# zlib-ng/minizip-ng

Measured on NVIDIA H100. Metric: deflate_l1_crc32_input_throughput, higher is better.
Workload: dtype u8

## Files before the change

minizip-ng_b200/csrc/deflate_kernel.cuh:

```cuda
#ifndef MZ_DEFLATE_KERNEL_CUH
#define MZ_DEFLATE_KERNEL_CUH

#include "mzcuda_common.cuh"

namespace mzc {

constexpr int DF_THREADS = 512;
constexpr int DF_WARPS = DF_THREADS / 32;
constexpr int DF_CHUNK_MAX = 65536;
constexpr int DF_UNIT = 32768;
constexpr int DF_SB = DF_UNIT;
constexpr int DF_SPAN = 8;
constexpr int DF_BATCH = DF_THREADS * DF_SPAN;
constexpr int DF_NBATCH = DF_UNIT / DF_BATCH;
constexpr int DF_MINMATCH = 4;
constexpr int DF_LOCKLEN = 8;
constexpr int DF_HASH_BITS = 13;
constexpr int DF_HASH_ENTRIES = 1 << DF_HASH_BITS;
constexpr int DF_STAGE_WORDS = DF_UNIT / 4 + 64;
constexpr int DF_HDR_WORDS = 96;

constexpr uint32_t DF_FLAG_FINAL = 1u;
constexpr uint32_t DF_FLAG_DICT = 2u;

constexpr int DF_OFF_IN = 0;
constexpr int DF_OFF_HASH = DF_OFF_IN + DF_UNIT + 64;
constexpr int DF_OFF_STAGE = DF_OFF_HASH;
constexpr int DF_OFF_REC = DF_OFF_HASH + DF_STAGE_WORDS * 4;
constexpr int DF_OFF_SPN = DF_OFF_REC + DF_NBATCH * DF_THREADS * 8;
constexpr int DF_SPAN_BYTES = DF_NBATCH * DF_THREADS * 10;
constexpr int DF_OFF_HIST = DF_OFF_REC + DF_SPAN_BYTES;
constexpr int DF_OFF_HIST2 = DF_OFF_HIST + (288 + 32) * 4;
constexpr int DF_OFF_CODE = DF_OFF_HIST2 + 256 * 4;
constexpr int DF_OFF_LENS = DF_OFF_CODE + (288 + 32) * 4;
constexpr int DF_OFF_BITS = DF_OFF_LENS + (288 + 32);
constexpr int DF_OFF_SCAN = DF_OFF_BITS + (288 + 32);
constexpr int DF_OFF_BB = DF_OFF_SCAN + 256 * 4;
constexpr int DF_OFF_MISC = DF_OFF_BB + 512 * 4;
constexpr int DF_OFF_SINK = DF_OFF_MISC + 32 * 4 + 16;
constexpr int DF_OFF_LSYM = DF_OFF_SINK + 32 * 4;
constexpr int DF_SMEM_BYTES = DF_OFF_LSYM + 256 * 2;
constexpr int DF_OFF_CAPL = DF_OFF_HIST;
static_assert(DF_OFF_CAPL + DF_WARPS * DF_NBATCH * 32 <= DF_OFF_SCAN, "capped-span lists fit in front of the scan scratch");
constexpr uint32_t DF_ZERO_SYM = 286;
static_assert(DF_HASH_ENTRIES * 4 <= DF_STAGE_WORDS * 4, "hash fits the staging region");
constexpr int DFH_PREV = 32768;
constexpr int DFH_HASH_BITS = 14;
constexpr int DFH_OFF_HASH = (DF_SMEM_BYTES + 15) & ~15;
constexpr int DFH_SMEM_BYTES = DFH_PREV + DFH_OFF_HASH + (4 << DFH_HASH_BITS);
static_assert(DFH_SMEM_BYTES <= 227 * 1024, "shared memory budget of the history variant");
static_assert(DF_SMEM_BYTES <= 113 * 1024, "shared memory budget for two CTAs per SM");

enum { MISC_CHUNK = 3, MISC_CARRY = 8  };

struct DeflateParams {
    const uint8_t *in;
    const uint64_t *in_off;
    const uint32_t *in_len;
    const uint8_t *flags;
    uint64_t total_len;
    uint32_t chunk_size;
    uint32_t nchunks;
    uint32_t last_flags;
    int32_t level;
    uint8_t *out;
    uint64_t slot_stride;
    uint32_t *out_len;
    uint32_t *work_counter;
};

__host__ __device__ inline uint64_t deflate_slot_bound(uint32_t chunk_size) {
    return (((uint64_t)chunk_size + 12ull * ((chunk_size + DF_SB - 1) / DF_SB + 1) + 64 + 15) & ~15ull);
}

__device__ __forceinline__ void length_symbol(uint32_t len, uint32_t &sym, uint32_t &ebits, uint32_t &eval) {
    const uint32_t l = len - 3;
    const uint32_t msb = 31u - (uint32_t)__clz((int)(l | 4u));
    uint32_t e = msb - 2;
    uint32_t sy = 4 * (e + 1) + ((l >> e) & 3u);
    uint32_t ev = l & ((1u << e) - 1u);
    sy = l < 8 ? l : sy;
    const bool top = len == 258;
    sym = top ? 28u : sy;
    ebits = top ? 0u : e;
    eval = top ? 0u : ev;
}
__device__ __forceinline__ void dist_symbol0(uint32_t d, uint32_t &sym, uint32_t &ebits) {
    uint32_t m = 31u - (uint32_t)__clz((int)(d | 1u));
    ebits = m > 0 ? m - 1 : 0u;
    sym = 2 * m + ((d >> ebits) & 1u);
}
__device__ __forceinline__ uint32_t len_extra_bits(uint32_t lsym) { return (lsym < 8 || lsym >= 28) ? 0u : (lsym >> 2) - 1; }
__device__ __forceinline__ uint32_t dist_extra_bits(uint32_t dsym) { return dsym < 4 ? 0u : (dsym >> 1) - 1; }

__device__ __forceinline__ uint32_t stage_word(uint32_t base, uint32_t pos, uint32_t k4) { return base + __umulhi(pos, 1u << 27) * k4; }

__device__ __forceinline__ void stage_put(uint32_t *stage, uint32_t pos, uint32_t v, uint32_t n) {
    if (n == 0) return;
    if (n < 32) v &= (1u << n) - 1;
    uint32_t w = pos >> 5, s = pos & 31;
    atomicOr(&stage[w], v << s);
    if (s + n > 32) atomicOr(&stage[w + 1], v >> (32 - s));
}

__device__ __forceinline__ void stage_or(const Smem &sm, uint32_t pos, uint32_t v, uint32_t n) {
    const uint32_t sh = pos & 31u, wa = DF_OFF_STAGE + ((pos >> 5) << 2);
    sm.red_or32(wa, v << sh);
    if (sh + n > 32) sm.red_or32(wa + 4, v >> (32 - sh));
}

struct BitWriter {
    Smem sm;
    uint64_t acc;
    uint32_t nb, wa;
    __device__ __forceinline__ void init(const Smem &s, uint32_t bitoff) {
        sm = s; wa = DF_OFF_STAGE + (bitoff >> 5) * 4; nb = bitoff & 31; acc = 0;
    }
    __device__ __forceinline__ void put(uint32_t v, uint32_t n) {
        acc |= (uint64_t)v << nb;
        nb += n;
        if (nb >= 32) {
            sm.red_or32(wa, (uint32_t)acc);
            acc >>= 32; nb -= 32; wa += 4;
        }
    }
    __device__ __forceinline__ uint32_t bitpos() const { return ((wa - (uint32_t)DF_OFF_STAGE) << 3) + nb; }
    __device__ __forceinline__ void finish() {
        if (nb > 0) sm.red_or32(wa, (uint32_t)acc);
        if (nb > 32) sm.red_or32(wa + 4, (uint32_t)(acc >> 32));
    }
};

enum { DF_PH_LOAD, DF_PH_PARSE, DF_PH_M0, DF_PH_COVER, DF_PH_T_M1, DF_PH_D, DF_PH_EMIT, DF_PH_FLUSH, DF_PH_UNITS,
       DF_PH_D_STATS, DF_PH_D_SWEEP1, DF_PH_D_SWEEP2, DF_PH_D_KRAFT, DF_PH_D_CANON, DF_PH_D_PASSES,
       DF_PH_P_A = DF_PH_D_PASSES + 8, DF_PH_P_B, DF_PH_P_C, DF_PH_M_INDEX, DF_PH_M_NEAR, DF_PH_M_EXTEND, DF_PH_X_SCAN, DF_PH_X_EMIT,
       DF_PH_X_M3, DF_PH_COLS };
constexpr int DF_PH_ROWS = 1024;
#if defined(MZ_DF_PHASES) && !defined(MZ_EMU)
__device__ unsigned long long g_df_phases[DF_PH_ROWS][DF_PH_COLS];
#define DF_PHASE_BEGIN(t) unsigned long long t = clock64()
#define DF_PHASE(t, ph)                                                                        \
    do {                                                                                       \
        if (threadIdx.x == 0 && blockIdx.x < (unsigned)DF_PH_ROWS) {                           \
            const unsigned long long now_ = clock64();                                         \
            atomicAdd(&g_df_phases[blockIdx.x][ph], now_ - (t));                               \
            if ((ph) == DF_PH_LOAD) atomicAdd(&g_df_phases[blockIdx.x][DF_PH_UNITS], 1ull);   \
            (t) = now_;                                                                        \
        }                                                                                      \
    } while (0)
#define DF_PHASE_COUNT(col)                                                                                          \
    do {                                                                                                             \
        if (threadIdx.x == 0 && blockIdx.x < (unsigned)DF_PH_ROWS) atomicAdd(&g_df_phases[blockIdx.x][col], 1ull); \
    } while (0)
#else
#define DF_PHASE_BEGIN(t)
#define DF_PHASE(t, ph)
#define DF_PHASE_COUNT(col)
#endif

constexpr int DF_BB_THREADS = 320;
enum { BB_STAT = 0 , BB_KRAFT = 8 , BB_SLACK = 136 ,
       BB_CNTW = 144 ,
       BB_NZ = 464 , BB_ST = 474 ,
       BB_HSUM = 484 , BB_HDRBITS = 494 ,
       BB_TOKBITS = 495 , BB_TOKW = 496  };

constexpr uint64_t CL_LENS = 0x12ddad91b725bb4ull;
constexpr uint64_t CL_CODE_LO = 0x840013930ef3c6ull, CL_CODE_HI = 0xd5c7fdf6cb149ull;
constexpr uint64_t CL_ORDER57 = 0x1b6d6db248db92dull;
__device__ __forceinline__ uint32_t cl_len(uint32_t s) { return (uint32_t)(CL_LENS >> (3 * s)) & 7u; }
__device__ __forceinline__ uint32_t cl_code(uint32_t s) {
    return s < 10 ? (uint32_t)(CL_CODE_LO >> (6 * s)) & 63u : (uint32_t)(CL_CODE_HI >> (6 * (s - 10))) & 63u;
}

__device__ __forceinline__ void bb_count_lengths(uint32_t *cntw_row, uint32_t L, unsigned lane, unsigned &m) {
    if (lane < 16) cntw_row[lane] = 0;
    __syncwarp();
    m = __match_any_sync(MZ_FULL_MASK, L);
    if (L > 0 && lane == (unsigned)(__ffs((int)m) - 1)) cntw_row[L] = (uint32_t)__popc(m);
    __syncwarp();
}

__device__ inline void block_build_codes(const uint32_t *hist_ll, const uint32_t *hist_lit2, const uint32_t *hist_d, uint8_t *lens_ll, uint8_t *lens_d,
                                         uint32_t *code_ll, uint32_t *code_d, uint8_t *bits_ll, uint8_t *bits_d, uint32_t *bb,
                                         uint32_t *stage, uint32_t hdrpos, uint32_t bfinal) {
    const uint32_t tid = threadIdx.x;
    const unsigned lane = lane_id(), w = warp_id();
    const int a = tid < 288 ? 0 : (tid < 320 ? 1 : 2);
    const uint32_t sym = a == 0 ? tid : tid - 288;
    const uint32_t nsym = a == 0 ? 286u : 30u;
    const int M = 15;
    const uint32_t one = 1u << M;
    const uint32_t w0 = a == 0 ? 0u : 9u;
    uint32_t c = (a < 2 && sym < nsym) ? (a == 0 ? hist_ll[sym] + (sym < 256 ? hist_lit2[sym] : 0u) : hist_d[sym]) : 0u;
    DF_PHASE_BEGIN(d_t);

    if (tid < 144) bb[tid] = (tid == BB_STAT + 2 || tid == BB_STAT + 6) ? 0xffffffffu : 0u;
    bar_sync(1, DF_BB_THREADS);
    if (a < 2) {
        uint32_t used_w = __reduce_add_sync(MZ_FULL_MASK, c ? 1u : 0u);
        uint32_t tot_w = __reduce_add_sync(MZ_FULL_MASK, c);
        uint32_t first_w = __reduce_min_sync(MZ_FULL_MASK, c ? sym : 0xffffffffu);
        if (lane == 0) {
            atomicAdd(&bb[BB_STAT + a * 4 + 0], used_w);
            atomicAdd(&bb[BB_STAT + a * 4 + 1], tot_w);
            atomicMin(&bb[BB_STAT + a * 4 + 2], first_w);
        }
    }
    bar_sync(1, DF_BB_THREADS);
    DF_PHASE(d_t, DF_PH_D_STATS);
    float ideal = 0.f;
    if (a < 2) {
        uint32_t used = bb[BB_STAT + a * 4 + 0], total = bb[BB_STAT + a * 4 + 1], fu = bb[BB_STAT + a * 4 + 2];
        if (used < 2) {
            uint32_t d0 = used == 0 ? 0u : (fu == 0 ? 1u : 0u);
            uint32_t d1 = used == 0 ? 1u : d0;
            if ((sym == d0 || sym == d1) && c == 0) c = 1;
            total += 2 - used;
        }
        if (c) ideal = __log2f((float)total) - __log2f((float)c);
    }
    float lo = -3.0f, step = 0.25f;
    uint32_t slack[2] = {0, 0};
    for (int sweep = 0; sweep < 2; sweep++) {
        if (a < 2) {
            uint32_t mine = 0;
#pragma unroll
            for (int cnd = 0; cnd < 16; cnd++) {
                uint32_t kr = 0;
                if (c) {
                    int l = (int)ceilf(ideal - (lo + step * (float)cnd));
                    l = l < 1 ? 1 : (l > M ? M : l);
                    kr = 1u << (M - l);
                }
                kr = __reduce_add_sync(MZ_FULL_MASK, kr);
                mine = lane == (unsigned)cnd ? kr : mine;
            }
            if (lane < 16) atomicAdd(&bb[BB_KRAFT + sweep * 32 + a * 16 + lane], mine);
        }
        bar_sync(1, DF_BB_THREADS);
        DF_PHASE(d_t, DF_PH_D_SWEEP1 + sweep);
        const uint32_t kl = bb[BB_KRAFT + sweep * 32 + lane];
        const unsigned fit = __ballot_sync(MZ_FULL_MASK, (lane & 15u) != 0 && kl <= one);
        const int best0 = (fit & 0xffffu) ? 31 - __clz((int)(fit & 0xffffu)) : 0;
        const int best1 = (fit >> 16) ? 31 - __clz((int)(fit >> 16)) : 0;
        slack[0] = one - __shfl_sync(MZ_FULL_MASK, kl, best0);
        slack[1] = one - __shfl_sync(MZ_FULL_MASK, kl, 16 + best1);
        lo = lo + step * (float)(a == 0 ? best0 : best1);
        step *= 0.0625f;
    }
    uint32_t L = 0;
    if (c) {
        int l = (int)ceilf(ideal - lo);
        L = (uint32_t)(l < 1 ? 1 : (l > M ? M : l));
    }
    unsigned m = 0;
    int buf = 0, pass = 0;
    bool settled = false;
    for (; pass < 40; pass++) {
        if (slack[0] == 0 && slack[1] == 0) break;
        uint32_t *cntw = bb + BB_CNTW + buf * 160, *nxt = bb + BB_CNTW + (buf ^ 1) * 160;
        if (a < 2) bb_count_lengths(cntw + w * 16, L, lane, m);
        bar_sync(1, DF_BB_THREADS);
        if (w == 0 || w == 9) {
            const int aa = w == 0 ? 0 : 1;
            const uint32_t wa = aa == 0 ? 0u : 9u, wb = aa == 0 ? 9u : 10u;
            const bool mine = lane >= 1 && lane <= (unsigned)M;
            uint32_t P[9], tot = 0;
#pragma unroll
            for (int i = 0; i < 9; i++) {
                const uint32_t t = (mine && wa + i < wb) ? cntw[(wa + i) * 16 + lane] : 0u;
                P[i] = tot;
                tot += t;
            }
            uint32_t sl = slack[aa], myk = 0;
            for (int len = 2; len <= M; len++) {
                uint32_t t = __shfl_sync(MZ_FULL_MASK, tot, len);
                uint32_t can = sl >> (M - len);
                uint32_t k = t < can ? t : can;
                if (lane == (unsigned)len) myk = k;
                sl -= k << (M - len);
            }
            const uint32_t kup = __shfl_down_sync(MZ_FULL_MASK, myk, 1);
            const uint32_t tot2 = mine ? tot - myk + kup : 0u;
            uint32_t code = 0, prev = 0, mycode = 0;
            for (int len = 1; len <= M; len++) {
                code = (code + prev) << 1;
                if (lane == (unsigned)len) mycode = code;
                prev = __shfl_sync(MZ_FULL_MASK, tot2, len);
// ... 162 lines not shown
__device__ __forceinline__ uint32_t opaque4() { return blockDim.x / (uint32_t)(DF_THREADS / 4); }

template <bool HIST>
__device__ __forceinline__ uint32_t hash_addr(uint32_t v, uint32_t k4) {
    return (HIST ? DFH_OFF_HASH : DF_OFF_HASH) + __umulhi(v * 2654435761u, 1u << (HIST ? DFH_HASH_BITS : DF_HASH_BITS)) * k4;
}

__device__ __forceinline__ uint32_t rec_len(uint32_t r) { uint32_t l = (r >> 3) & 255u; return l ? l + 3 : 0u; }

__device__ __forceinline__ uint32_t fin_len(uint32_t m) { return ((m >> 4) & 255u) + 3u; }
__device__ __forceinline__ uint32_t fin_dist(uint32_t m) { return ((m >> 12) & 0x7fffu) + 1u; }
template <bool ONEM>
__device__ __forceinline__ void span_classify(const Smem &sm, uint32_t A, uint32_t B, uint32_t q0, uint32_t cover, uint32_t &F, uint32_t &MA,
                                              uint32_t &MB) {
    const uint32_t lit = (A >> 26) | ((B >> 26) << 6);
    const uint32_t crel = cover > q0 ? cover - q0 : 0u;
    const uint32_t cr8 = crel < 8 ? crel : 8u;
    uint32_t ex = 0;
    MA = MB = 0;
#pragma unroll
    for (int r = 0; r < (ONEM ? 1 : 2); r++) {
        const uint32_t R = r == 0 ? A : B;
        const uint32_t j = R & 7u, end = j + rec_len(R);
        const uint32_t s = j > crel ? j : crel;
        const uint32_t Lf = (end > s ? end : s) - s;
        const uint32_t P = (s < 8u ? s : 8u) & 7u;
        const uint32_t M = Lf >= 3 ? (((Lf << 4) + (0x80000000u - (3u << 4))) | P | ((R << 1) & (0x7fffu << 12))) : 0u;
        if (r == 0) MA = M;
        else MB = M;
        ex = Lf - 1u < 2u ? Lf : ex;
    }
    F = ((lit >> cr8) << cr8) | (ex << 8);
    if (ex) {
        const uint32_t p = DF_OFF_IN + q0 + crel;
        F |= sm.ld8(p) << 16;
        if (ex == 2) F |= sm.ld8(p + 1) << 24;
    }
}

__device__ __forceinline__ uint32_t match_symbols(const Smem &sm, uint32_t M) {
    uint32_t ds, db;
    const uint32_t lsv = sm.ld16(DF_OFF_LSYM + ((M >> 3) & 0x1feu));
    const uint32_t d = fin_dist(M) - 1;
    dist_symbol0(d, ds, db);
    sm.red_add32(DF_OFF_HIST + (257u + (lsv & 31u)) * 4, 1u);
    sm.red_add32(DF_OFF_HIST + (288u + ds) * 4, 1u);
    return 0x80000000u | ((M & 7u) << 28) | ((d & ((1u << db) - 1u)) << 15) | (ds << 10) | lsv;
}
__device__ __forceinline__ uint32_t match_bits(const Smem &sm, uint32_t M) {
    const uint32_t n = sm.ld8(DF_OFF_BITS + 257u + (M & 31u)) + sm.ld8(DF_OFF_BITS + 288u + ((M >> 10) & 31u));
    return M ? n : 0u;
}
__device__ __forceinline__ void put_match_bits(const Smem &sm, uint32_t pos, uint32_t M) {
    const uint32_t cwl = sm.ld32(DF_OFF_CODE + (257u + (M & 31u)) * 4);
    const uint32_t cwd = sm.ld32(DF_OFF_CODE + (288u + ((M >> 10) & 31u)) * 4);
    const uint32_t cl = (cwl >> 16) & 15u, cd = (cwd >> 16) & 15u;
    const uint32_t v1 = (cwl & 0x7fffu) | (((M >> 5) & 31u) << cl);
    const uint32_t n1 = cl + ((cwl >> 20) & 15u);
    const uint32_t v2 = (cwd & 0x7fffu) | (((M >> 15) & 0x1fffu) << cd);
    const uint64_t V = (uint64_t)v1 | ((uint64_t)v2 << n1);
    const uint32_t lo = (uint32_t)V, hi = (uint32_t)(V >> 32);
    const uint32_t wa = stage_word(DF_OFF_STAGE, pos, opaque4());
    const uint32_t w0 = __funnelshift_l(0u, lo, pos), w1 = __funnelshift_l(lo, hi, pos), w2 = __funnelshift_l(hi, 0u, pos);
    sm.red_or32(wa, w0);
    sm.red_or32(wa + 4, w1);
    if (w2) sm.red_or32(wa + 8, w2);
}

__device__ __forceinline__ uint32_t nth_parked(const uint32_t (&bm)[DF_NBATCH], uint32_t k, uint32_t warp) {
    uint32_t r = k, word = 0, bsel = 0;
    bool found = false;
#pragma unroll
    for (int b = 0; b < DF_NBATCH; b++) {
        const uint32_t c = (uint32_t)__popc(bm[b]);
        const bool here = !found && r < c;
        word = here ? bm[b] : word;
        bsel = here ? (uint32_t)b : bsel;
        found = found || here;
        r -= found ? 0u : c;
    }
    uint32_t base = 0;
#pragma unroll
    for (int st = 16; st; st >>= 1) {
        const uint32_t c = (uint32_t)__popc((word >> base) & ((1u << st) - 1u));
        const bool up = r >= c;
        r -= up ? c : 0u;
        base += up ? (uint32_t)st : 0u;
    }
    return found ? bsel * (uint32_t)DF_THREADS + warp * 32u + base : 0xffffffffu;
}

struct SpanBits {
    uint32_t v[4], E0, E1, offs, xv, MA, size;
};
template <bool ONEM>
__device__ __forceinline__ SpanBits span_bits(const Smem &sm, uint32_t sidx, uint32_t F, uint32_t MA, uint32_t MB, uint32_t code_base, uint32_t zero_ent,
                                              uint32_t k4) {
    SpanBits s;
    const uint2 x = sm.ld64(DF_OFF_IN + sidx * DF_SPAN);
    uint32_t xn = 0;
    s.xv = 0;
    const uint32_t ex = (F >> 8) & 3u;
    if (ex) {
        const uint32_t c0 = sm.ld32(DF_OFF_CODE + ((F >> 16) & 0xffu) * 4);
        s.xv = c0 & 0x7fffu;
        xn = (c0 >> 16) & 15u;
        if (ex == 2) {
            const uint32_t c1 = sm.ld32(DF_OFF_CODE + (F >> 24) * 4);
            s.xv |= (c1 & 0x7fffu) << xn;
            xn += (c1 >> 16) & 15u;
        }
    }
    uint32_t cw[8];
#pragma unroll
    for (int j = 0; j < 8; j++) {
        const uint32_t by = MZ_BYTE(j < 4 ? x.x : x.y, j & 3);
        cw[j] = sm.ld32_a(((F >> j) & 1u) ? by * k4 + code_base : zero_ent);
    }
    const uint32_t nA = match_bits(sm, MA), nB = ONEM ? 0u : match_bits(sm, MB);
    const uint32_t sA = MA ? ((MA >> 28) & 7u) * 8u : 64u, sB = MB ? ((MB >> 28) & 7u) * 8u : 64u;
    const uint32_t L0 = __byte_perm(__byte_perm(cw[0], cw[1], 0x0062u), __byte_perm(cw[2], cw[3], 0x0062u), 0x5410u) + shl_clamp(nA, sA) + shl_clamp(nB, sB);
    const uint32_t L1 = __byte_perm(__byte_perm(cw[4], cw[5], 0x0062u), __byte_perm(cw[6], cw[7], 0x0062u), 0x5410u) + shl_clamp(nA, sA - 32u) + shl_clamp(nB, sB - 32u);
    const uint32_t P0 = L0 * 0x01010101u;
    const uint32_t P1 = L1 * 0x01010101u + (P0 >> 24) * 0x01010101u;
    s.E0 = P0 << 8;
    s.E1 = __funnelshift_l(P0, P1, 8);
#pragma unroll
    for (int jj = 0; jj < 4; jj++) {
        const uint32_t c0 = cw[2 * jj], c1 = cw[2 * jj + 1];
        s.v[jj] = (c0 & 0xffffu) | ((c1 & 0xffffu) << (c0 >> 16));
    }
    s.offs = xn + (((shr_clamp(s.E0, sA) & 0xffu) + (shr_clamp(s.E1, sA - 32u) & 0xffu)) << 8) +
             (((shr_clamp(s.E0, sB) & 0xffu) + (shr_clamp(s.E1, sB - 32u) & 0xffu)) << 16);
    s.MA = MA;
    s.size = xn + (P1 >> 24);
    return s;
}
template <bool ONEM>
__device__ __forceinline__ void span_emit(const Smem &sm, const SpanBits &s, uint32_t pos, uint32_t sidx, uint32_t stage_base, uint32_t k4) {
    const uint32_t xn = s.offs & 0xffu;
    if (xn) stage_or(sm, pos, s.xv, xn);
    pos += xn;
#pragma unroll
    for (int jj = 0; jj < 4; jj++) {
        const uint32_t pp = pos + MZ_BYTE(jj < 2 ? s.E0 : s.E1, 2 * (jj & 1));
        const uint32_t wa = stage_word(stage_base, pp, k4);
        sm.red_or32_a(wa, __funnelshift_l(0u, s.v[jj], pp));
        sm.red_or32_a(wa + 4, __funnelshift_l(s.v[jj], 0u, pp));
    }
    if (s.MA) put_match_bits(sm, pos + ((s.offs >> 8) & 0xffu), s.MA);
    if (!ONEM) sm.st32(DF_OFF_REC + sidx * 8, pos + (s.offs >> 16));
}

template <int STRIDE, bool LAZY, bool HIST = false>
__global__ void __launch_bounds__(DF_THREADS, HIST ? 1 : 2) deflate_chunks_kernel(DeflateParams P) {
    MZ_DYN_SMEM(smem_raw);
    uint8_t *const smem = smem_raw + (HIST ? DFH_PREV : 0);
    constexpr uint32_t CUR = HIST ? (uint32_t)DFH_PREV : 0u;
    uint8_t *s_in = smem + DF_OFF_IN;
    uint32_t *s_stage = (uint32_t *)(smem + DF_OFF_STAGE);
    uint32_t *s_hist_ll = (uint32_t *)(smem + DF_OFF_HIST);
    uint32_t *s_hist_d = s_hist_ll + 288;
    uint32_t *s_code_ll = (uint32_t *)(smem + DF_OFF_CODE);
    uint32_t *s_code_d = s_code_ll + 288;
    uint8_t *s_lens_ll = smem + DF_OFF_LENS;
    uint8_t *s_lens_d = s_lens_ll + 288;
    uint8_t *s_bits_ll = smem + DF_OFF_BITS;
    uint8_t *s_bits_d = s_bits_ll + 288;
    uint32_t *s_scan = (uint32_t *)(smem + DF_OFF_SCAN);
    uint32_t *s_bb = (uint32_t *)(smem + DF_OFF_BB);
    uint32_t *s_misc = (uint32_t *)(smem + DF_OFF_MISC);
#ifndef MZ_EMU
    uint64_t *s_bar = (uint64_t *)(smem + DF_OFF_MISC + 32 * 4);
    uint32_t bar_phase = 0;
    if (threadIdx.x == 0) {
        mbar_init(s_bar, 1);
        mbar_fence_init();
    }
    __syncthreads();
#endif
    const uint32_t tid = threadIdx.x;
    const unsigned lane = lane_id(), warp = warp_id();
    Smem sm;
    sm.init(smem);
    if (tid < 256) {
        uint32_t ls, lb, lv;
        length_symbol(tid + 3, ls, lb, lv);
        sm.st16(DF_OFF_LSYM + tid * 2, ls | (lv << 5));
    }
    constexpr bool ONEM = false;
    DF_PHASE_BEGIN(ph_t);

    for (uint32_t chunk_static = blockIdx.x;; chunk_static += gridDim.x) {
        uint32_t chunk = chunk_static;
        if (P.work_counter) {
            if (tid == 0) s_misc[MISC_CHUNK] = atomicAdd(P.work_counter, 1u);
            __syncthreads();
            chunk = s_misc[MISC_CHUNK];
        }
        if (chunk >= P.nchunks) {
            if (P.work_counter && tid == 0 && atomicAdd(P.work_counter + 1, 1u) == gridDim.x - 1) {
                P.work_counter[0] = 0;
                P.work_counter[1] = 0;
            }
            break;
        }
        uint64_t off;
        uint32_t len, flags;
        if (P.in_off) {
            off = P.in_off[chunk];
            len = P.in_len[chunk];
            flags = P.flags ? P.flags[chunk] : 0u;
        } else {
            off = (uint64_t)chunk * P.chunk_size;
            uint64_t rem = P.total_len - off;
            len = rem < P.chunk_size ? (uint32_t)rem : P.chunk_size;
            flags = P.flags ? P.flags[chunk] : ((chunk == P.nchunks - 1 ? P.last_flags & ~DF_FLAG_DICT : 0u) | (P.last_flags & DF_FLAG_DICT));
        }
        const bool dict = HIST && (flags & DF_FLAG_DICT) && off >= (uint64_t)DFH_PREV;
        uint8_t *gout = P.out + (uint64_t)chunk * P.slot_stride;

        uint32_t flushed = 0;
        uint32_t bitpos = 0;
        const uint32_t nunits = (len + DF_UNIT - 1) / DF_UNIT;
        if (tid < 4) s_misc[MISC_CARRY + tid] = 0;

        if (len == 0) {
            for (uint32_t i = tid; i < 64; i += DF_THREADS) s_stage[i] = 0;
            __syncthreads();
            if (flags & DF_FLAG_FINAL) {
                if (tid == 0) stage_put(s_stage, 0, 1u | (1u << 1), 3);
                bitpos = 10;
            }
            __syncthreads();
        }

        for (uint32_t u = 0; u < nunits; u++) {
            const uint32_t ustart = u * DF_UNIT;
            const uint32_t ulen = (ustart + DF_UNIT < len) ? (uint32_t)DF_UNIT : len - ustart;
            const uint8_t *gin = P.in + off + ustart;
            const bool last_unit = u == nunits - 1;
            const uint32_t nb = (ulen + DF_BATCH - 1) / DF_BATCH;

            const uint32_t len16 = ulen & ~15u;
            bool bulk = false;
#ifndef MZ_EMU
            bulk = (((uintptr_t)gin) & 15) == 0 && len16 > 0;
            if (bulk && tid == 0) {
                fence_proxy_async();
                mbar_expect_tx(s_bar, len16);
                tma_load_1d(s_in, gin, len16, s_bar);
            }
#endif
            if (!bulk) {
                if ((((uintptr_t)gin) & 15) == 0) {
                    for (uint32_t i = tid * 16; i < len16; i += DF_THREADS * 16) *(uint4 *)(s_in + i) = ldg_stream((const uint4 *)(gin + i));
                } else {
                    for (uint32_t i = tid; i < len16; i += DF_THREADS) s_in[i] = gin[i];
                }
            }
            for (uint32_t i = len16 + tid; i < ulen; i += DF_THREADS) s_in[i] = gin[i];
            for (uint32_t i = ulen + tid; i < ((ulen + 63) & ~15u) + 16 && i < DF_UNIT + 64; i += DF_THREADS) s_in[i] = 0;
            if (P.level != 0) {
                if (!HIST) {
                    for (uint32_t i = tid; i < DF_HASH_ENTRIES / 4; i += DF_THREADS) sm.st128(DF_OFF_HASH + i * 16, ~0u, ~0u, ~0u, ~0u);
                } else if (u == 0) {
                    for (uint32_t i = tid; i < (1u << DFH_HASH_BITS) / 4; i += DF_THREADS) sm.st128(DFH_OFF_HASH + i * 16, ~0u, ~0u, ~0u, ~0u);
                    if (dict) {
                        const uint8_t *gp = P.in + off - DFH_PREV;
                        if ((((uintptr_t)gp) & 15) == 0) {
                            for (uint32_t i = tid * 16; i < (uint32_t)DFH_PREV; i += DF_THREADS * 16) *(uint4 *)(smem - DFH_PREV + i) = ldg_stream((const uint4 *)(gp + i));
                        } else {
                            for (uint32_t i = tid; i < (uint32_t)DFH_PREV; i += DF_THREADS) smem[(int)i - DFH_PREV] = gp[i];
                        }
                    }
                } else {
                    for (uint32_t i = tid; i < (1u << DFH_HASH_BITS) / 4; i += DF_THREADS) {
                        uint4 e = *(const uint4 *)(smem + DFH_OFF_HASH + i * 16);
                        e.x = (e.x != ~0u && (e.x & 0xffffu) >= (uint32_t)DFH_PREV) ? e.x + 0x78000u : ~0u;
                        e.y = (e.y != ~0u && (e.y & 0xffffu) >= (uint32_t)DFH_PREV) ? e.y + 0x78000u : ~0u;
                        e.z = (e.z != ~0u && (e.z & 0xffffu) >= (uint32_t)DFH_PREV) ? e.z + 0x78000u : ~0u;
                        e.w = (e.w != ~0u && (e.w & 0xffffu) >= (uint32_t)DFH_PREV) ? e.w + 0x78000u : ~0u;
                        *(uint4 *)(smem + DFH_OFF_HASH + i * 16) = e;
                    }
                }
            }
#ifndef MZ_EMU
            if (bulk) {
                mbar_wait(s_bar, bar_phase);
                bar_phase ^= 1;
            }
#endif
            __syncthreads();
            if (HIST && P.level != 0 && u == 0 && dict) {
#pragma unroll 1
                for (uint32_t b = 0; b < (uint32_t)DF_NBATCH; b++) {
                    const uint32_t p0 = b * DF_BATCH + tid * DF_SPAN;
                    const uint2 x = sm.ld64((uint32_t)(DF_OFF_IN - DFH_PREV) + p0);
                    const uint32_t y = sm.ld32((uint32_t)(DF_OFF_IN - DFH_PREV) + p0 + 8);
                    const uint32_t key0 = ((15u - b) << 16) | p0;
#pragma unroll
                    for (int j = 0; j < 8; j++) {
                        const uint32_t v = j == 0 ? x.x : (j < 4 ? __funnelshift_r(x.x, x.y, 8 * j) : (j == 4 ? x.y : __funnelshift_r(x.y, y, 8 * (j - 4))));
                        sm.red_min32(hash_addr<true>(v, 4u), key0 + j);
                    }
                }
                __syncthreads();
            }
            DF_PHASE(ph_t, DF_PH_LOAD);

            uint32_t fF[DF_NBATCH], fA[DF_NBATCH];
            bool stored = (P.level == 0);
            const uint32_t bfinal = (last_unit && (flags & DF_FLAG_FINAL)) ? 1u : 0u;

            if (P.level != 0) {
                DF_PHASE_BEGIN(p_t);
                uint32_t ncap = 0;
#pragma unroll 1
                for (uint32_t b = 0; b < nb; b++) {
                    const uint32_t q0 = b * DF_BATCH + tid * DF_SPAN;
                    uint32_t v[12], ha[8], lc[8];
                    const uint32_t k4 = opaque4();
                    {
                        const uint2 x = sm.ld64(DF_OFF_IN + q0), y = sm.ld64(DF_OFF_IN + q0 + 8);
                        v[0] = x.x; v[4] = x.y; v[8] = y.x;
#pragma unroll
                        for (int k = 1; k < 4; k++) {
                            v[k] = __funnelshift_r(x.x, x.y, 8 * k);
                            v[4 + k] = __funnelshift_r(x.y, y.x, 8 * k);
                            v[8 + k] = __funnelshift_r(y.x, y.y, 8 * k);
                        }
                    }
#pragma unroll
                    for (int j = 0; j < 8; j++) {
                        ha[j] = hash_addr<HIST>(v[j], k4);
                        if (j % STRIDE == 0) lc[j] = sm.ld32(ha[j]);
                    }
                    const uint32_t nvalid = ulen > q0 ? (ulen - q0 < 8 ? ulen - q0 : 8u) : 0u;
                    __syncthreads();
                    DF_PHASE(p_t, DF_PH_P_A);
                    const uint32_t key0 = ((uint32_t)(DF_NBATCH - 1 - b) << 16) | (CUR + q0);
#pragma unroll
                    for (int j = 0; j < 8; j++) sm.red_min32(ha[j], key0 + j);
                    __syncthreads();
                    DF_PHASE(p_t, DF_PH_P_B);
#pragma unroll
                    for (int j = 0; j < 8; j++) {
                        if (j % STRIDE != 0) {
                            lc[j] = 0;
                            continue;
                        }
                        const uint32_t kp = key0 + j, kn = sm.ld32(ha[j]);
                        const uint32_t ck = kn < kp ? kn : lc[j];
                        const uint32_t c = HIST ? ck & 0xffffu : ck;
                        const uint32_t ca = DF_OFF_IN - CUR + (c & 0xfffcu);
                        const uint32_t w0 = sm.ld32(ca), w1 = sm.ld32(ca + 4), w2 = sm.ld32(ca + 8);
                        const uint32_t s = c << 3;
                        const uint32_t x0 = __funnelshift_r(w0, w1, s) ^ v[j];
                        const uint32_t x1 = __funnelshift_r(w1, w2, s) ^ v[j + 4];
                        const bool reach = HIST ? c < CUR + q0 + j && c >= q0 + j : ck != 0xffffffffu;
                        const uint32_t l3 = ((uint32_t)__clz((int)__brev(x1)) & ~7u) + 8u;
                        lc[j] = sel_u32(reach && x0 == 0, (((kp - ck - 1u) << 11) & (0x7fffu << 11)) + l3 + (uint32_t)j, 0u);
                    }
                    if (q0 + 16 > ulen) {
#pragma unroll
                        for (int j = 0; j < 8; j += STRIDE) {
                            const uint32_t room = ulen > q0 + j ? ulen - (q0 + j) : 0u;
                            const uint32_t l = rec_len(lc[j]);
                            lc[j] = l >= (uint32_t)DF_MINMATCH && l > room ? (room >= (uint32_t)DF_MINMATCH ? lc[j] - ((l - room) << 3) : 0u) : lc[j];
                        }
                    }
                    uint32_t nxt = 0, lit = 0, mA = 0, mB = 0, span_end = 0;
                    if (STRIDE == 2 && !LAZY && !ONEM) {
#pragma unroll
                        for (int j = 6; j >= 0; j -= 2) mA = lc[j] ? lc[j] : mA;
                        const uint32_t endA = (mA & 7u) + rec_len(mA);
#pragma unroll
                        for (int j = 6; j >= 2; j -= 2) mB = lc[j] && (uint32_t)j >= endA ? lc[j] : mB;
                        const uint32_t endB = (mB & 7u) + rec_len(mB);
                        lit = ~(((1u << endA) - (1u << (mA & 7u))) | ((1u << endB) - (1u << (mB & 7u)))) & 0xffu;
                        span_end = mB ? endB : endA;
                    } else {
#pragma unroll
                        for (int j = 0; j < 8; j++) {
                            const bool take = nxt == (uint32_t)j;
                            if (j % STRIDE == 0) {
                                const uint32_t rec = lc[j], l = rec_len(rec);
                                bool ism = take && rec != 0;
                                if (LAZY && STRIDE == 1 && j < 7) ism = ism && !(((lc[j + 1] >> 3) & 255u) > ((rec >> 3) & 255u));
                                const bool first = mA == 0;
                                if (ONEM) ism = ism && first;
                                mA = (ism && first) ? rec : mA;
                                if (!ONEM) mB = (ism && !first) ? rec : mB;
                                lit |= (take && !ism) ? (1u << j) : 0u;
                                nxt = ism ? (uint32_t)j + l : (take ? (uint32_t)j + 1u : nxt);
                            } else {
                                lit |= take ? (1u << j) : 0u;
                                nxt = take ? (uint32_t)j + 1u : nxt;
                            }
                        }
                        const uint32_t last = mB ? mB : mA;
                        span_end = last ? (last & 7u) + rec_len(last) : 0u;
                    }
                    lit &= (1u << nvalid) - 1u;
                    {
                        const uint32_t last = mB ? mB : mA;
                        const bool cap = ((last >> 3) & 255u) == (uint32_t)(DF_LOCKLEN - 3);
                        const uint32_t capped = __ballot_sync(MZ_FULL_MASK, cap);
                        sm.st8_if(cap, DF_OFF_CAPL + warp * 256u + ncap + (uint32_t)__popc(capped & ((1u << lane) - 1u)), (b << 5) | lane);
                        ncap += (uint32_t)__popc(capped);
                        sm.st64(DF_OFF_REC + (b * DF_THREADS + tid) * 8, mA | ((lit & 63u) << 26), mB | ((lit >> 6) << 26));
                        sm.st16(DF_OFF_SPN + (b * DF_THREADS + tid) * 2, ((last & 7u) << 9) | span_end);
                    }
                    DF_PHASE(p_t, DF_PH_P_C);
                }
                DF_PHASE(ph_t, DF_PH_PARSE);
                {
                    DF_PHASE_BEGIN(m_t);
                    __syncwarp();
                    for (uint32_t k0 = 0; k0 < ncap; k0 += 32) {
                        const uint32_t k = k0 + lane;
                        const uint32_t e = k < ncap ? sm.ld8(DF_OFF_CAPL + warp * 256u + k) : 0u;
                        const uint32_t sidx = (e >> 5) * (uint32_t)DF_THREADS + warp * 32u + (e & 31u);
                        DF_PHASE(m_t, DF_PH_M_INDEX);
                        if (k < ncap) {
                            const uint2 r = sm.ld64(DF_OFF_REC + sidx * 8);
                            const bool second = (r.y & 0x03ffffffu) != 0;
                            const uint32_t w = second ? r.y : r.x, last = w & 0x03ffffffu;
                            const uint32_t j = last & 7u, q = sidx * DF_SPAN + j, c = q - ((last >> 11) & 0x7fffu) - 1u;
                            uint32_t maxlen = ulen - q;
                            maxlen = maxlen < 258 ? maxlen : 258u;
                            uint32_t l = 0, cb = c;
                            if (q >= 4) {
                                const uint32_t a0 = sm.ld32u(DF_OFF_IN, q), a1 = sm.ld32u(DF_OFF_IN, q + 4);
                                const bool p4 = a0 == a1, p3 = __funnelshift_r(a0, a1, 24) == a0;
                                if (p4 || p3) {
                                    uint32_t cn = c;
                                    if (p4) {
                                        if (a0 == sm.ld32u(DF_OFF_IN, q - 4)) cn = q - 4;
                                        if (a0 == sm.ld32u(DF_OFF_IN, q - 2)) cn = q - 2;
                                        if (a0 == sm.ld32u(DF_OFF_IN, q - 1)) cn = q - 1;
                                    } else if (a0 == sm.ld32u(DF_OFF_IN, q - 3) && a1 == sm.ld32u(DF_OFF_IN, q + 1)) {
                                        cn = q - 3;
                                    }
                                    if (cn != c) {
                                        const uint32_t pd = q - cn;
                                        if (q >= 12u && (sidx & 31u) != 0u && sm.ld32u(DF_OFF_IN, q - 8) == sm.ld32u(DF_OFF_IN, q - 8 - pd) &&
                                            sm.ld32u(DF_OFF_IN, q - 4) == sm.ld32u(DF_OFF_IN, q - 4 - pd)) {
                                            const uint32_t left = ulen - sidx * DF_SPAN, nval = left < 8u ? left : 8u;
                                            const uint32_t lit = ((r.x >> 26) | ((r.y >> 26) << 6) | (0xffu << j)) & ((1u << nval) - 1u);
                                            const uint32_t mA = second ? (r.x & 0x03ffffffu) : 0u;
                                            sm.st64(DF_OFF_REC + sidx * 8, mA | ((lit & 63u) << 26), (lit >> 6) << 26);
                                            sm.st16(DF_OFF_SPN + sidx * 2, mA ? ((mA & 7u) << 9) | ((mA & 7u) + rec_len(mA)) : 0u);
                                            continue;
                                        }
                                        l = extend_match8(sm, cn, q, maxlen);
                                        cb = cn;
                                    }
                                }
                            }
                            DF_PHASE(m_t, DF_PH_M_NEAR);
                            if (l < 64u && l < maxlen) {
                                const uint32_t lf = extend_match8(sm, c, q, maxlen);
                                if (lf > l) {
                                    l = lf;
                                    cb = c;
                                }
                            }
                            sm.st32(DF_OFF_REC + sidx * 8 + (second ? 4u : 0u), (w & ~((255u << 3) | (0x7fffu << 11))) | ((l - 3) << 3) | ((q - cb - 1u) << 11));
                            sm.st16(DF_OFF_SPN + sidx * 2, (j << 9) | (j + l));
                            DF_PHASE(m_t, DF_PH_M_EXTEND);
                        }
                    }
                }
                __syncthreads();
                DF_PHASE(ph_t, DF_PH_M0);

                for (uint32_t i = tid; i < DF_STAGE_WORDS / 4; i += DF_THREADS) {
                    if (i == 0) sm.st128(DF_OFF_STAGE, s_misc[MISC_CARRY], s_misc[MISC_CARRY + 1], s_misc[MISC_CARRY + 2], s_misc[MISC_CARRY + 3]);
                    else sm.st128(DF_OFF_STAGE + i * 16, 0, 0, 0, 0);
                }
                for (uint32_t i = tid; i < 288 + 32 + 256; i += DF_THREADS) s_hist_ll[i] = 0;

                {
                    uint32_t se[8];
                    if (tid * 8 < nb * DF_THREADS) {
                        const uint4 q = *(const uint4 *)(smem + DF_OFF_SPN + tid * 16);
                        se[0] = q.x & 0xffffu; se[1] = q.x >> 16; se[2] = q.y & 0xffffu; se[3] = q.y >> 16;
                        se[4] = q.z & 0xffffu; se[5] = q.z >> 16; se[6] = q.w & 0xffffu; se[7] = q.w >> 16;
                    } else {
#pragma unroll
                        for (int k = 0; k < 8; k++) se[k] = 0;
                    }
                    const uint32_t p0 = tid * 64;
                    uint32_t tmax = 0;
#pragma unroll
                    for (int k = 0; k < 8; k++) {
                        const uint32_t e = se[k] ? p0 + 8 * k + (se[k] & 511u) : 0u;
                        tmax = tmax > e ? tmax : e;
                    }
                    const uint32_t incl = warp_incl_max(tmax);
                    uint32_t cin = __shfl_up_sync(MZ_FULL_MASK, incl, 1);
                    if (lane == 0) cin = 0;
                    if (lane == 31) s_scan[warp] = incl;
                    __syncthreads();
                    {
                        const uint32_t w = (lane < (unsigned)DF_WARPS && lane < warp) ? s_scan[lane] : 0u;
                        const uint32_t base = __reduce_max_sync(MZ_FULL_MASK, w);
                        cin = cin > base ? cin : base;
                    }
                    uint32_t run = cin, drop = 0, pcv = 0, pendk = 0;
                    bool alive = false;
                    uint32_t cv[8];
#pragma unroll
                    for (int k = 0; k < 8; k++) {
                        const uint32_t q0 = p0 + 8 * k;
                        const uint32_t ms = q0 + (se[k] >> 9), me = q0 + (se[k] & 511u);
                        const bool fc = run >= q0 + 8;
                        const bool strad = se[k] != 0 && ms < run && me > run;
                        const bool takes = fc && strad && alive && ms <= pcv;
                        drop |= takes ? 1u << pendk : 0u;
                        cv[k] = takes ? pcv : run;
                        pcv = (fc && strad && !takes) ? run : pcv;
                        pendk = (fc && strad) ? (uint32_t)k : pendk;
                        alive = fc && (strad || alive);
                        run = (se[k] != 0 && me > run) ? me : run;
                    }
#pragma unroll
                    for (int k = 0; k < 8; k++) cv[k] = ((drop >> k) & 1u) ? 0xffffu : cv[k];
                    *(uint4 *)(smem + DF_OFF_SPN + tid * 16) = make_uint4(cv[0] | (cv[1] << 16), cv[2] | (cv[3] << 16), cv[4] | (cv[5] << 16), cv[6] | (cv[7] << 16));
                }
                __syncthreads();
                DF_PHASE(ph_t, DF_PH_COVER);

                const uint32_t hist_lit = sm.addr((lane & 1u) ? (uint32_t)DF_OFF_HIST2 : (uint32_t)DF_OFF_HIST);
                const uint32_t k4 = opaque4();
                const uint32_t sink = sm.addr(DF_OFF_SINK + lane * 4);
                uint32_t bmB[DF_NBATCH];
#pragma unroll
                for (int b = 0; b < DF_NBATCH; b++) {
                    uint32_t F = 0, MA = 0, MB = 0;
                    bmB[b] = 0;
                    if ((uint32_t)b < nb) {
                        const uint32_t sidx = (uint32_t)b * DF_THREADS + tid;
                        const uint32_t q0 = sidx * DF_SPAN;
                        const uint2 r = sm.ld64(DF_OFF_REC + sidx * 8);
                        const uint32_t cover = sm.ld16(DF_OFF_SPN + sidx * 2);
                        span_classify<ONEM>(sm, r.x, r.y, q0, cover, F, MA, MB);
                        const uint32_t ex = (F >> 8) & 3u;
                        if (ex) {
                            sm.red_add32_a(hist_lit + ((F >> 16) & 0xffu) * 4, 1u);
                            if (ex == 2) sm.red_add32_a(hist_lit + (F >> 24) * 4, 1u);
                        }
                        const uint2 x = sm.ld64(DF_OFF_IN + q0);
#pragma unroll
                        for (int j = 0; j < 8; j++) {
                            const uint32_t by = MZ_BYTE(j < 4 ? x.x : x.y, j & 3);
                            sm.red_add32_a(((F >> j) & 1u) ? by * k4 + hist_lit : sink, 1u);
                        }
                        if (MA) MA = match_symbols(sm, MA);
                        if (!ONEM) {
                            bmB[b] = __ballot_sync(MZ_FULL_MASK, MB != 0);
                            sm.st32(DF_OFF_REC + sidx * 8 + 4, MB);
                        }
                    }
                    fF[b] = F; fA[b] = MA;
                }
                if (!ONEM) {
                    uint32_t totB = 0;
#pragma unroll
                    for (int b = 0; b < DF_NBATCH; b++) totB += (uint32_t)__popc(bmB[b]);
                    __syncwarp();
                    for (uint32_t k0 = 0; k0 < totB; k0 += 32) {
                        const uint32_t sidx = nth_parked(bmB, k0 + lane, warp);
                        if (sidx != 0xffffffffu) {
                            const uint32_t a = DF_OFF_REC + sidx * 8 + 4;
                            sm.st32(a, match_symbols(sm, sm.ld32(a)));
                        }
                    }
                }
                if (tid == 0) sm.red_add32(DF_OFF_HIST + 256 * 4, 1u);
                __syncthreads();
                DF_PHASE(ph_t, DF_PH_T_M1);
#ifdef MZ_DF_CODES_HOOK
                if (tid == 0) MZ_DF_CODES_HOOK(s_hist_ll, (const uint32_t *)(smem + DF_OFF_HIST2), s_hist_d);
#endif
                if (tid < DF_BB_THREADS)
                    block_build_codes(s_hist_ll, (const uint32_t *)(smem + DF_OFF_HIST2), s_hist_d, s_lens_ll, s_lens_d, s_code_ll, s_code_d, s_bits_ll, s_bits_d, s_bb,
                                      s_stage, bitpos, bfinal);
                __syncthreads();
                DF_PHASE(ph_t, DF_PH_D);
                const uint32_t hdrbits = s_bb[BB_HDRBITS], tokbits = s_bb[BB_TOKBITS];
                const uint32_t eob = s_code_ll[256];
                const uint32_t dyn_bits = hdrbits + tokbits + ((eob >> 16) & 15u);
                const uint32_t stored_bits = (((bitpos + 3 + 7) & ~7u) - bitpos) + 32 + ulen * 8;
                if (dyn_bits >= stored_bits) {
                    stored = true;
                    const uint32_t w0 = bitpos >> 5;
                    for (uint32_t i = tid; i <= (hdrbits + 31) / 32 + 1; i += DF_THREADS)
                        s_stage[w0 + i] = i == 0 ? s_stage[w0] & ((1u << (bitpos & 31u)) - 1u) : 0u;
                    __syncthreads();
                } else {
                    const uint32_t code_base = sm.addr(DF_OFF_CODE), zero_ent = sm.addr(DF_OFF_CODE + DF_ZERO_SYM * 4), stage_base = sm.addr(DF_OFF_STAGE);
                    const uint32_t k4 = opaque4();
                    uint32_t run = bitpos + hdrbits;
                    DF_PHASE_BEGIN(x_t);
#pragma unroll
                    for (int b = 0; b < DF_NBATCH; b += 2) {
                        if ((uint32_t)b >= nb) break;
                        const uint32_t s0 = (uint32_t)b * DF_THREADS + tid, s1 = s0 + DF_THREADS;
                        const uint32_t MB0 = ONEM ? 0u : sm.ld32(DF_OFF_REC + s0 * 8 + 4);
                        const uint32_t MB1 = (ONEM || (uint32_t)b + 1 >= nb) ? 0u : sm.ld32(DF_OFF_REC + s1 * 8 + 4);
                        const SpanBits A = span_bits<ONEM>(sm, s0, fF[b], fA[b], MB0, code_base, zero_ent, k4);
                        const SpanBits B = span_bits<ONEM>(sm, s1, fF[b + 1], fA[b + 1], MB1, code_base, zero_ent, k4);
                        const uint32_t sz = A.size | (B.size << 16);
                        const uint32_t incl = warp_incl_sum(sz);
                        if (lane == 31) s_scan[(b / 2) * DF_WARPS + warp] = incl;
                        __syncthreads();
                        DF_PHASE(x_t, DF_PH_X_SCAN);
                        const uint32_t wt = lane < (unsigned)DF_WARPS ? s_scan[(b / 2) * DF_WARPS + lane] : 0u;
                        const uint32_t wlo = wt & 0xffffu, whi = wt >> 16;
                        const uint32_t totA = __reduce_add_sync(MZ_FULL_MASK, wlo);
                        const uint32_t ex = incl - sz;
                        const uint32_t posA = run + __reduce_add_sync(MZ_FULL_MASK, lane < warp ? wlo : 0u) + (ex & 0xffffu);
                        const uint32_t posB = run + totA + __reduce_add_sync(MZ_FULL_MASK, lane < warp ? whi : 0u) + (ex >> 16);
                        run += totA + __reduce_add_sync(MZ_FULL_MASK, whi);
                        if (A.size) span_emit<ONEM>(sm, A, posA, s0, stage_base, k4);
                        if (B.size) span_emit<ONEM>(sm, B, posB, s1, stage_base, k4);
                        DF_PHASE(x_t, DF_PH_X_EMIT);
                    }
#ifdef MZ_EMU
                    if (run != bitpos + hdrbits + tokbits) {
                        fprintf(stderr, "deflate: block %u, unit %u: emitted %u token bits, the histograms count %u\n", (unsigned)blockIdx.x, u,
                                run - bitpos - hdrbits, tokbits);
                        abort();
                    }
#endif
                    if (!ONEM) {
                        uint32_t totB = 0;
#pragma unroll
                        for (int b = 0; b < DF_NBATCH; b++) totB += (uint32_t)__popc(bmB[b]);
                        __syncwarp();
                        for (uint32_t k0 = 0; k0 < totB; k0 += 32) {
                            const uint32_t sidx = nth_parked(bmB, k0 + lane, warp);
                            if (sidx != 0xffffffffu) {
                                const uint2 r = sm.ld64(DF_OFF_REC + sidx * 8);
                                put_match_bits(sm, r.x, r.y);
                            }
                        }
                    }
                    DF_PHASE(x_t, DF_PH_X_M3);
                    if (tid == DF_THREADS - 1) stage_put(s_stage, bitpos + hdrbits + tokbits, eob & 0x7fffu, (eob >> 16) & 15u);
                    bitpos += dyn_bits;
                }
            } else {
                for (uint32_t i = tid; i < DF_STAGE_WORDS / 4; i += DF_THREADS) {
                    if (i == 0) sm.st128(DF_OFF_STAGE, s_misc[MISC_CARRY], s_misc[MISC_CARRY + 1], s_misc[MISC_CARRY + 2], s_misc[MISC_CARRY + 3]);
                    else sm.st128(DF_OFF_STAGE + i * 16, 0, 0, 0, 0);
                }
                __syncthreads();
            }
            if (stored) {
                const uint32_t p0 = (bitpos + 3 + 7) >> 3;
                if (tid == 0) {
                    stage_put(s_stage, bitpos, bfinal, 3);
                    stage_put(s_stage, p0 * 8, ulen, 16);
                    stage_put(s_stage, p0 * 8 + 16, ulen ^ 0xffffu, 16);
                }
                for (uint32_t i = tid * 4; i < ulen; i += DF_THREADS * 4) {
                    uint32_t v = load32u(s_in, i);
                    uint32_t n = ulen - i;
                    stage_put(s_stage, (p0 + 4 + i) * 8, v, n >= 4 ? 32 : n * 8);
                }
                bitpos = (p0 + 4 + ulen) * 8;
            }
            __syncthreads();
            DF_PHASE(ph_t, DF_PH_EMIT);
            {
                const uint32_t n16 = bitpos >> 7;
                const uint32_t used_words = (bitpos + 31) >> 5;
#pragma unroll 4
                for (uint32_t i = tid; i < n16; i += DF_THREADS) ((uint4 *)(gout + flushed))[i] = ((const uint4 *)s_stage)[i];
                if (tid < 4) s_misc[MISC_CARRY + tid] = (n16 * 4 + tid < used_words) ? s_stage[n16 * 4 + tid] : 0u;
                bitpos -= n16 * 128;
                flushed += n16 * 16;
                if (HIST && u + 1 < nunits)
                    for (uint32_t i = tid; i < (uint32_t)DF_UNIT / 16; i += DF_THREADS) *(uint4 *)(smem - DFH_PREV + i * 16) = *(const uint4 *)(s_in + i * 16);
                __syncthreads();
                DF_PHASE(ph_t, DF_PH_FLUSH);
            }
        }


        {
            if (tid < 8) {
                const uint32_t v = tid < 4 ? (len == 0 ? s_stage[tid] : s_misc[MISC_CARRY + tid]) : 0u;
                __syncwarp(0xffu);
                s_stage[tid] = v;
            }
            __syncthreads();
            if (flags & DF_FLAG_FINAL) {
                bitpos = (bitpos + 7) & ~7u;
            } else {
                const uint32_t p0 = (bitpos + 3 + 7) >> 3;
                if (tid == 0) stage_put(s_stage, (p0 + 2) * 8, 0xffffu, 16);
                bitpos = (p0 + 4) * 8;
            }
            __syncthreads();
            if (tid < 8) ((uint32_t *)(gout + flushed))[tid] = s_stage[tid];
            if (tid == 0) P.out_len[chunk] = flushed + (bitpos >> 3);
            __syncthreads();
            DF_PHASE(ph_t, DF_PH_FLUSH);
        }
    }
}

__host__ __device__ inline int deflate_stride_for_level(int level) { return level <= 1 ? 2 : 1; }
__host__ __device__ inline bool deflate_lazy_for_level(int level) { return level >= 4; }
__host__ __device__ inline bool deflate_hist_for_level(int level) { return level >= 6; }

}
#endif
```

Before: 161.9.

## Prefetch next unit's input via TMA during flush and pre-claim next chunk

After emitting a unit, thread 0 issues the bulk TMA load of the next unit (or the next chunk's first unit) into s_in while the block flushes the staged output. It claims the next chunk from the work counter early, overlapping the atomic with code building. This is meant to hide global-to-shared load latency behind the output flush. It also moves the nvalid mask computation into the tail-only path and trims one loop iteration in the tail match selection. The cost is more bookkeeping in shared misc slots and some risk of ordering bugs if s_in is overwritten while still being read.

```diff
diff --git a/minizip-ng_b200/csrc/deflate_kernel.cuh b/minizip-ng_b200/csrc/deflate_kernel.cuh
--- a/minizip-ng_b200/csrc/deflate_kernel.cuh
+++ b/minizip-ng_b200/csrc/deflate_kernel.cuh
@@ -51,7 +51,7 @@
 static_assert(DFH_SMEM_BYTES <= 227 * 1024, "shared memory budget of the history variant");
 static_assert(DF_SMEM_BYTES <= 113 * 1024, "shared memory budget for two CTAs per SM");
 
-enum { MISC_CHUNK = 3, MISC_CARRY = 8  };
+enum { MISC_NEXT_CHUNK = 2, MISC_CHUNK = 3, MISC_NEXT = 4 , MISC_PRE = 7, MISC_CARRY = 8  };
 
 struct DeflateParams {
     const uint8_t *in;
@@ -134,7 +134,7 @@
 enum { DF_PH_LOAD, DF_PH_PARSE, DF_PH_M0, DF_PH_COVER, DF_PH_T_M1, DF_PH_D, DF_PH_EMIT, DF_PH_FLUSH, DF_PH_UNITS,
        DF_PH_D_STATS, DF_PH_D_SWEEP1, DF_PH_D_SWEEP2, DF_PH_D_KRAFT, DF_PH_D_CANON, DF_PH_D_PASSES,
        DF_PH_P_A = DF_PH_D_PASSES + 8, DF_PH_P_B, DF_PH_P_C, DF_PH_M_INDEX, DF_PH_M_NEAR, DF_PH_M_EXTEND, DF_PH_X_SCAN, DF_PH_X_EMIT,
-       DF_PH_X_M3, DF_PH_COLS };
+       DF_PH_X_M3, DF_PH_L_RESET, DF_PH_COLS };
 constexpr int DF_PH_ROWS = 1024;
 #if defined(MZ_DF_PHASES) && !defined(MZ_EMU)
 __device__ unsigned long long g_df_phases[DF_PH_ROWS][DF_PH_COLS];
@@ -603,6 +603,35 @@
     if (!ONEM) sm.st32(DF_OFF_REC + sidx * 8, pos + (s.offs >> 16));
 }
 
+__device__ __forceinline__ void chunk_extent(const DeflateParams &P, uint32_t chunk, uint64_t &off, uint32_t &len) {
+    if (P.in_off) {
+        off = P.in_off[chunk];
+        len = P.in_len[chunk];
+    } else {
+        off = (uint64_t)chunk * P.chunk_size;
+        const uint64_t rem = P.total_len - off;
+        len = rem < P.chunk_size ? (uint32_t)rem : P.chunk_size;
+    }
+}
+
+__device__ __forceinline__ uint32_t unit_bulk_bytes(const uint8_t *gin, uint32_t ulen) {
+    return (((uintptr_t)gin) & 15) == 0 ? ulen & ~15u : 0u;
+}
+
+__device__ __forceinline__ void unit_load_bulk(const Smem &sm, uint8_t *s_in, const uint8_t *gin, uint32_t n16, uint64_t *bar) {
+#ifndef MZ_EMU
+    fence_proxy_async();
+    mbar_expect_tx(bar, n16);
+    tma_load_1d(s_in, gin, n16, bar);
+#else
+    (void)s_in; (void)bar;
+    for (uint32_t i = 0; i < n16; i += 16) {
+        const uint4 v = *(const uint4 *)(gin + i);
+        sm.st128(DF_OFF_IN + i, v.x, v.y, v.z, v.w);
+    }
+#endif
+}
+
 template <int STRIDE, bool LAZY, bool HIST = false>
 __global__ void __launch_bounds__(DF_THREADS, HIST ? 1 : 2) deflate_chunks_kernel(DeflateParams P) {
     MZ_DYN_SMEM(smem_raw);
@@ -621,15 +650,17 @@
     uint32_t *s_scan = (uint32_t *)(smem + DF_OFF_SCAN);
     uint32_t *s_bb = (uint32_t *)(smem + DF_OFF_BB);
     uint32_t *s_misc = (uint32_t *)(smem + DF_OFF_MISC);
+    uint64_t *s_bar = (uint64_t *)(smem + DF_OFF_MISC + 32 * 4);
+    bool have_chunk = false;
+    if (threadIdx.x == 0) s_misc[MISC_PRE] = 0;
 #ifndef MZ_EMU
-    uint64_t *s_bar = (uint64_t *)(smem + DF_OFF_MISC + 32 * 4);
     uint32_t bar_phase = 0;
     if (threadIdx.x == 0) {
         mbar_init(s_bar, 1);
         mbar_fence_init();
     }
+#endif
     __syncthreads();
-#endif
     const uint32_t tid = threadIdx.x;
     const unsigned lane = lane_id(), warp = warp_id();
     Smem sm;
@@ -645,7 +676,8 @@
     for (uint32_t chunk_static = blockIdx.x;; chunk_static += gridDim.x) {
         uint32_t chunk = chunk_static;
         if (P.work_counter) {
-            if (tid == 0) s_misc[MISC_CHUNK] = atomicAdd(P.work_counter, 1u);
+            if (tid == 0 && !have_chunk) s_misc[MISC_CHUNK] = atomicAdd(P.work_counter, 1u);
+            have_chunk = false;
             __syncthreads();
             chunk = s_misc[MISC_CHUNK];
         }
@@ -658,14 +690,10 @@
         }
         uint64_t off;
         uint32_t len, flags;
+        chunk_extent(P, chunk, off, len);
         if (P.in_off) {
-            off = P.in_off[chunk];
-            len = P.in_len[chunk];
             flags = P.flags ? P.flags[chunk] : 0u;
         } else {
-            off = (uint64_t)chunk * P.chunk_size;
-            uint64_t rem = P.total_len - off;
-            len = rem < P.chunk_size ? (uint32_t)rem : P.chunk_size;
             flags = P.flags ? P.flags[chunk] : ((chunk == P.nchunks - 1 ? P.last_flags & ~DF_FLAG_DICT : 0u) | (P.last_flags & DF_FLAG_DICT));
         }
         const bool dict = HIST && (flags & DF_FLAG_DICT) && off >= (uint64_t)DFH_PREV;
@@ -693,15 +721,21 @@
             const bool last_unit = u == nunits - 1;
             const uint32_t nb = (ulen + DF_BATCH - 1) / DF_BATCH;
 
+            DF_PHASE_BEGIN(l_t);
             const uint32_t len16 = ulen & ~15u;
-            bool bulk = false;
+            const uint32_t n16 = unit_bulk_bytes(gin, ulen);
+            const bool fetched = !HIST && n16 != 0 && s_misc[MISC_PRE] != 0;
+            if (!HIST && tid == 0) {
+                const uint64_t g = (uint64_t)(uintptr_t)(gin + ulen);
+                s_misc[MISC_NEXT] = (uint32_t)g;
+                s_misc[MISC_NEXT + 1] = (uint32_t)(g >> 32);
+                s_misc[MISC_NEXT + 2] = len - ustart - ulen;
+            }
 #ifndef MZ_EMU
-            bulk = (((uintptr_t)gin) & 15) == 0 && len16 > 0;
-            if (bulk && tid == 0) {
-                fence_proxy_async();
-                mbar_expect_tx(s_bar, len16);
-                tma_load_1d(s_in, gin, len16, s_bar);
-            }
+            const bool bulk = n16 != 0;
+            if (bulk && !fetched && tid == 0) unit_load_bulk(sm, s_in, gin, n16, s_bar);
+#else
+            const bool bulk = fetched;
 #endif
             if (!bulk) {
                 if ((((uintptr_t)gin) & 15) == 0) {
@@ -736,6 +770,7 @@
                     }
                 }
             }
+            DF_PHASE(l_t, DF_PH_L_RESET);
 #ifndef MZ_EMU
             if (bulk) {
                 mbar_wait(s_bar, bar_phase);
@@ -787,7 +822,6 @@
                         ha[j] = hash_addr<HIST>(v[j], k4);
                         if (j % STRIDE == 0) lc[j] = sm.ld32(ha[j]);
                     }
-                    const uint32_t nvalid = ulen > q0 ? (ulen - q0 < 8 ? ulen - q0 : 8u) : 0u;
                     __syncthreads();
                     DF_PHASE(p_t, DF_PH_P_A);
                     const uint32_t key0 = ((uint32_t)(DF_NBATCH - 1 - b) << 16) | (CUR + q0);
@@ -795,6 +829,7 @@
                     for (int j = 0; j < 8; j++) sm.red_min32(ha[j], key0 + j);
                     __syncthreads();
                     DF_PHASE(p_t, DF_PH_P_B);
+                    uint32_t vmask = 0xffu;
 #pragma unroll
                     for (int j = 0; j < 8; j++) {
                         if (j % STRIDE != 0) {
@@ -814,6 +849,8 @@
                         lc[j] = sel_u32(reach && x0 == 0, (((kp - ck - 1u) << 11) & (0x7fffu << 11)) + l3 + (uint32_t)j, 0u);
                     }
                     if (q0 + 16 > ulen) {
+                        const uint32_t nvalid = ulen > q0 ? (ulen - q0 < 8 ? ulen - q0 : 8u) : 0u;
+                        vmask = (1u << nvalid) - 1u;
 #pragma unroll
                         for (int j = 0; j < 8; j += STRIDE) {
                             const uint32_t room = ulen > q0 + j ? ulen - (q0 + j) : 0u;
@@ -827,9 +864,9 @@
                         for (int j = 6; j >= 0; j -= 2) mA = lc[j] ? lc[j] : mA;
                         const uint32_t endA = (mA & 7u) + rec_len(mA);
 #pragma unroll
-                        for (int j = 6; j >= 2; j -= 2) mB = lc[j] && (uint32_t)j >= endA ? lc[j] : mB;
+                        for (int j = 6; j >= 4; j -= 2) mB = lc[j] && (uint32_t)j >= endA ? lc[j] : mB;
                         const uint32_t endB = (mB & 7u) + rec_len(mB);
-                        lit = ~(((1u << endA) - (1u << (mA & 7u))) | ((1u << endB) - (1u << (mB & 7u)))) & 0xffu;
+                        lit = ~(((1u << endA) - (1u << (mA & 7u))) | ((1u << endB) - (1u << (mB & 7u)))) & vmask;
                         span_end = mB ? endB : endA;
                     } else {
 #pragma unroll
@@ -852,8 +889,8 @@
                         }
                         const uint32_t last = mB ? mB : mA;
                         span_end = last ? (last & 7u) + rec_len(last) : 0u;
-                    }
-                    lit &= (1u << nvalid) - 1u;
+                        lit &= vmask;
+                    }
                     {
                         const uint32_t last = mB ? mB : mA;
                         const bool cap = ((last >> 3) & 255u) == (uint32_t)(DF_LOCKLEN - 3);
@@ -1039,6 +1076,8 @@
                 if (tid < DF_BB_THREADS)
                     block_build_codes(s_hist_ll, (const uint32_t *)(smem + DF_OFF_HIST2), s_hist_d, s_lens_ll, s_lens_d, s_code_ll, s_code_d, s_bits_ll, s_bits_d, s_bb,
                                       s_stage, bitpos, bfinal);
+                else if (!HIST && tid == DF_THREADS - 1 && last_unit && P.work_counter)
+                    s_misc[MISC_NEXT_CHUNK] = atomicAdd(P.work_counter, 1u);
                 __syncthreads();
                 DF_PHASE(ph_t, DF_PH_D);
                 const uint32_t hdrbits = s_bb[BB_HDRBITS], tokbits = s_bb[BB_TOKBITS];
@@ -1127,6 +1166,28 @@
             }
             __syncthreads();
             DF_PHASE(ph_t, DF_PH_EMIT);
+            if (!HIST && tid == 0) {
+                const uint8_t *gnext = (const uint8_t *)(((uint64_t)s_misc[MISC_NEXT + 1] << 32) | s_misc[MISC_NEXT]);
+                uint32_t nlen = s_misc[MISC_NEXT + 2];
+                bool any = true;
+                if (nlen == 0) {
+                    const uint32_t nc = !P.work_counter ? chunk_static + gridDim.x
+                                                        : (P.level != 0 ? s_misc[MISC_NEXT_CHUNK] : atomicAdd(P.work_counter, 1u));
+                    if (P.work_counter) {
+                        s_misc[MISC_CHUNK] = nc;
+                        have_chunk = true;
+                    }
+                    any = nc < P.nchunks;
+                    if (any) {
+                        uint64_t noff;
+                        chunk_extent(P, nc, noff, nlen);
+                        gnext = P.in + noff;
+                    }
+                }
+                const uint32_t nn16 = any ? unit_bulk_bytes(gnext, nlen < (uint32_t)DF_UNIT ? nlen : (uint32_t)DF_UNIT) : 0u;
+                if (nn16) unit_load_bulk(sm, s_in, gnext, nn16, s_bar);
+                s_misc[MISC_PRE] = nn16;
+            }
             {
                 const uint32_t n16 = bitpos >> 7;
                 const uint32_t used_words = (bitpos + 31) >> 5;
```

After: 164.1, median of 6. 1.01x the previous value.
